# edp1096/toy-spice

Measured on NVIDIA B200. Metric: circuit-timesteps/sec (batched FP64 transient), higher is better.
Workload: dtype f64

## Files before the change

__graft_entry__.py:

```python
from __future__ import annotations

import importlib
import os
import re
import subprocess
import sys
from concurrent.futures import ThreadPoolExecutor

ROOT = os.path.dirname(os.path.abspath(__file__))
if ROOT not in sys.path:
    sys.path.insert(0, ROOT)

PKG = os.path.join(ROOT, "toy-spice_b200")
KCACHE = os.path.join(PKG, "_kcache")
NVCC = os.environ.get("NVCC", "/usr/local/cuda/bin/nvcc")
ARCH = ["-gencode", "arch=compute_100a,code=sm_100a"]


def _kernel_variants(T):
    W = importlib.import_module("toy-spice_b200.workloads")
    out = []

    def sweep_batch(ckt):
        b = ckt.batch(2)
        for (dev, par), vals in W.sweep_draws(ckt.devices(), 2, 1).items():
            b.set_param(dev, par, vals)
        return b

    for name, text in sorted(T.BUNDLED.items()):
        ckt = T.Circuit.from_netlist(text)
        out.append((name + ":nominal", ckt, ckt.batch(2)))
        out.append((name + ":sweep", ckt, sweep_batch(ckt)))
        card = ckt.analysis_card()
        if card["analysis"] == T.AN_DC:
            for label, b in ((":dc:nominal", ckt.batch(2)), (":dc:sweep", sweep_batch(ckt))):
                b.kernel_variant(card["dc_src_dev"])
                out.append((name + label, ckt, b))
    for k in (12, 24):
        ckt = T.Circuit.from_netlist(W.rc_ladder(k))
        out.append((f"ladder{k}:sweep", ckt, sweep_batch(ckt)))
    ckt = T.Circuit.from_netlist(W.diode_rc_ladder(24))
    out.append(("diodeladder24:sweep", ckt, sweep_batch(ckt)))
    try:
        sys.path.insert(0, os.path.join(ROOT, "tests"))
        extra = importlib.import_module("extra_decks").EXTRA
    except Exception:
        extra = {}
    for name, (text, an) in sorted(extra.items()):
        ckt = T.Circuit.from_netlist(text)
        out.append((name + ":sweep", ckt, sweep_batch(ckt)))
        if "dc" in an:
            cd = T.Circuit.from_netlist(an.get("dc_text", text))
            b = sweep_batch(cd)
            b.kernel_variant(an["dc"][0])
            out.append((name + ":dc:sweep", cd, b))
            if "dc_text" in an and an.get("op"):
                pass
        if "dc2" in an:
            b = sweep_batch(ckt)
            b.kernel_variant(an["dc2"][0][0], an["dc2"][1][0])
            out.append((name + ":dc2:sweep", ckt, b))
    try:
        acd = importlib.import_module("ac_decks")
        for name, text in sorted({**acd.AC_DECKS, **acd.AC_SINGULAR}.items()):
            ckt = T.Circuit.from_netlist(text)
            b = ckt.batch(2)
            for (dev, par), vals in acd.ac_draws(ckt.devices(), 2).items():
                b.set_param(dev, par, vals)
            out.append((name + ":ac", ckt, b))
    except Exception:
        pass
    return out

# ... 41 lines not shown
            break
    with open(os.path.join(KCACHE, autokey + ".auto"), "w") as f:
        f.write(f"{best}\n")
    return label, keys, status, best


def _coop_variants(T):
    out = []
    try:
        sys.path.insert(0, os.path.join(ROOT, "tests"))
        decks = dict(importlib.import_module("test_gpu_coop").DECKS)
        rd = importlib.import_module("random_decks")
        for k in (16,):
            decks[f"ladder{k}"] = (rd.rc_ladder(k), 0)
    except Exception as ex:
        print("[build] cooperative variants skipped:", ex)
        return out
    W = importlib.import_module("toy-spice_b200.workloads")
    for name, (text, _) in sorted(decks.items()):
        ckt = T.Circuit.from_netlist(text)
        b = ckt.batch(2)
        for (dev, par), vals in W.sweep_draws(ckt.devices(), 2, 1).items():
            b.set_param(dev, par, vals)
        out.append((f"{name}:thread:mb1", b, T.default_opts(strict_fp=0, min_blocks=1, coop_parts=0), ckt))
        for parts in (2, 4, 8):
            if ckt.coop_info(parts) is None:
                continue
            b = ckt.batch(2)
            for (dev, par), vals in W.sweep_draws(ckt.devices(), 2, 1).items():
                b.set_param(dev, par, vals)
            out.append((f"{name}:coop{parts}", b, T.default_opts(strict_fp=0, min_blocks=2, coop_parts=parts), ckt))
    ckt = T.Circuit.from_netlist(W.rc_ladder(32))
    b = ckt.batch(2)
    for (dev, par), vals in W.sweep_draws(ckt.devices(), 2, 1).items():
        b.set_param(dev, par, vals)
    out.append(("ladder32:thread:block96", b, T.default_opts(strict_fp=0, min_blocks=1, coop_parts=0, block_size=96), ckt))
    out.append(("ladder32:coop2", b, T.default_opts(strict_fp=0, min_blocks=2, coop_parts=2), ckt))
    return out


def _compile_coop(item):
    label, batch, opts, _ = item
    key = batch.kernel_key(opts)
    _, _, _, st = _nvcc_cubin(batch.kernel_source(opts), key, "true")
    return label, [key], st, 2


def build() -> None:
    subprocess.check_call(["make", "-C", os.path.join(PKG, "csrc"), "-s", "-j4"])
    T = importlib.import_module("toy-spice_b200")
    T.lib()
    os.makedirs(KCACHE, exist_ok=True)
    items = []
    seen = set()
    for label, ckt, batch in _kernel_variants(T):
        for strict in (0, 1):
            autokey = batch.kernel_key(T.default_opts(strict_fp=strict, min_blocks=0))
            if autokey in seen:
# ... 48 lines not shown
```

include/tspice_b200.h:

```cpp
#ifndef TSPICE_B200_H
#define TSPICE_B200_H

#include <stdint.h>

#ifdef __cplusplus
extern "C" {
#endif

typedef struct tsb_ctx tsb_ctx;
typedef struct tsb_plan tsb_plan;
typedef struct tsb_batch tsb_batch;
typedef struct tsb_job tsb_job;

enum {
    TSB_OK = 0,
    TSB_E_INVALID = -1,
    TSB_E_PARSE = -2,
    TSB_E_CUDA = -3,
    TSB_E_COMPILE = -4,
    TSB_E_UNSUPPORTED = -5,
    TSB_E_NOMEM = -6
};

enum {
// ... 129 lines not shown
int tsb_job_run_tran(tsb_job* job, double tstart, double tstop, double tstep, double tmax, int uic, int out_flags,
                     int64_t wave_cap_rows, const tsb_opts* opts);
int tsb_job_run_dc(tsb_job* job, int src_dev, double start, double stop, double inc, int out_flags, const tsb_opts* opts);
int tsb_job_sync(tsb_job* job);
int tsb_job_result_status(tsb_job* job, int32_t* status );
int tsb_job_result_rows(tsb_job* job, int64_t* rows );
int tsb_job_result_stats(tsb_job* job, double* stats );
int tsb_job_result_waveform(tsb_job* job, int64_t inst, double* out, int64_t cap_rows, int64_t* n_rows);
int tsb_job_result_summary(tsb_job* job, double* out, int64_t* rows_total, int64_t totals[5]);

int tsb_lu_order(int n, const double* A_nominal, int* pivot_row, int* pivot_col);
int tsb_batch_stamp_dev(tsb_batch* batch, int mode, double time, double dt, double gmin, uint64_t A_dev, uint64_t b_dev,
                        const tsb_opts* opts);
int tsb_lu_solve_batched(tsb_ctx* ctx, int n, const int* pivot_row, const int* pivot_col, const double* A, const double* b,
                         double* x, int32_t* status, int64_t n_inst, int strict_fp);
int tsb_lu_solve_batched_dev(tsb_ctx* ctx, int n, const int* pivot_row, const int* pivot_col, uint64_t A_dev, uint64_t b_dev,
                             uint64_t x_dev, uint64_t status_dev, int64_t n_inst, int strict_fp);
int tsb_lu_solve_batched_complex(tsb_ctx* ctx, int n, const int* pivot_row, const int* pivot_col, const double* A,
                                 const double* b, double* x, int32_t* status, int64_t n_inst, int strict_fp);
int tsb_lu_solve_batched_complex_dev(tsb_ctx* ctx, int n, const int* pivot_row, const int* pivot_col, uint64_t A_dev,
                                     uint64_t b_dev, uint64_t x_dev, uint64_t status_dev, int64_t n_inst, int strict_fp);

int tsb_batch_kernel_source(tsb_batch* batch, const tsb_opts* opts, char* buf, int64_t cap, int64_t* needed);
int tsb_batch_kernel_variant(tsb_batch* batch, int dc_src_dev, int dc_src2_dev, int grid);
int tsb_batch_kernel_key(tsb_batch* batch, const tsb_opts* opts, char* buf, int cap);
int64_t tsb_ctx_launch_count(const tsb_ctx* ctx);

#ifdef __cplusplus
}
#endif
#endif
```

toy-spice_b200/api.py:

```python
from __future__ import annotations

import ctypes as C
import os
import numpy as np

_HERE = os.path.dirname(os.path.abspath(__file__))
_LIB = None

AN_OP, AN_TRAN, AN_AC, AN_DC, AN_DC2 = 0, 1, 2, 3, 4
OUT_WAVE, OUT_STATS, OUT_GRID, OUT_AC_REFREAD = 1, 2, 4, 8
K_R, K_C, K_L, K_V, K_I, K_D, K_Q, K_M, K_K, K_LCORE = range(10)
ST_OK, ST_OP_FAILED, ST_TRAN_FAILED, ST_DC_FAILED, ST_OVERFLOW, ST_AC_FAILED = range(6)

ABI_SYMBOLS = [
    "tsb_default_opts", "tsb_version", "tsb_ctx_create", "tsb_ctx_destroy", "tsb_last_error", "tsb_ctx_set_stream",
    "tsb_ctx_set_cache_dir", "tsb_ctx_measure_fp64_peak", "tsb_ctx_sm_count", "tsb_plan_create",
    "tsb_plan_from_netlist", "tsb_plan_add_device", "tsb_plan_finalize", "tsb_plan_destroy", "tsb_plan_error",
    "tsb_plan_size", "tsb_plan_num_devices", "tsb_plan_device_info", "tsb_plan_device_params",
    "tsb_plan_find_device", "tsb_plan_node_name", "tsb_plan_analysis", "tsb_plan_structure", "tsb_plan_pattern",
    "tsb_plan_num_columns", "tsb_plan_column_name", "tsb_plan_coop_info", "tsb_batch_create", "tsb_batch_destroy", "tsb_batch_set_param",
    "tsb_batch_set_param_dev", "tsb_batch_set_param_uniform", "tsb_run_op", "tsb_run_tran", "tsb_run_dc",
    "tsb_batch_sync", "tsb_result_dims", "tsb_result_dev_ptrs", "tsb_result_rows", "tsb_result_status",
    "tsb_result_counters", "tsb_result_waveform", "tsb_result_wave_all", "tsb_result_stats_all",
    "tsb_result_totals", "tsb_batch_kernel_source", "tsb_batch_kernel_key", "tsb_ctx_launch_count",
# ... 402 lines not shown
        if np.isscalar(values):
            self._check(lib().tsb_batch_set_param_uniform(self.h, d, param, float(values)), "set_param_uniform")
            return
        if hasattr(values, "is_cuda") and values.is_cuda:
            import torch
            assert values.dtype == torch.float64 and values.is_contiguous() and values.numel() == self.n_inst
            self._keep[(d, param)] = values
            if self.ckt.ctx is not None:
                self.ckt.ctx.wait_torch_stream()
            self._check(lib().tsb_batch_set_param_dev(self.h, d, param, values.data_ptr()), "set_param_dev")
            return
        if hasattr(values, "numpy"):
            values = values.numpy()
        v = np.ascontiguousarray(values, dtype=np.float64)
        if v.shape != (self.n_inst,):
            raise ValueError("values must have shape [n_inst]")
        if zero_copy:
            self._keep[(d, param)] = v
            self._check(lib().tsb_batch_set_param_async(self.h, d, param, v.ctypes.data_as(C.POINTER(C.c_double))), "set_param_async")
        else:
            self._keep.pop((d, param), None)
            self._check(lib().tsb_batch_set_param(self.h, d, param, v.ctypes.data_as(C.POINTER(C.c_double))), "set_param")

    def kernel_variant(self, dc_src=-1, dc_src2=-1, grid=False):
        d1 = self._dev(dc_src) if dc_src != -1 else -1
        d2 = self._dev(dc_src2) if dc_src2 != -1 else -1
        self._check(lib().tsb_batch_kernel_variant(self.h, d1, d2, int(bool(grid))), "tsb_batch_kernel_variant")

    def kernel_source(self, opts: Opts | None = None) -> str:
        need = C.c_int64()
        o = C.byref(opts) if opts is not None else None
        lib().tsb_batch_kernel_source(self.h, o, None, 0, C.byref(need))
        buf = C.create_string_buffer(need.value)
        lib().tsb_batch_kernel_source(self.h, o, buf, need.value, C.byref(need))
        return buf.value.decode()

    def kernel_key(self, opts: Opts | None = None) -> str:
        buf = C.create_string_buffer(64)
        lib().tsb_batch_kernel_key(self.h, C.byref(opts) if opts is not None else None, buf, 64)
        return buf.value.decode()

    def run_op(self, opts: Opts | None = None):
        self._check(lib().tsb_run_op(self.h, C.byref(opts) if opts is not None else None), "tsb_run_op")

    def run_tran(self, tstart, tstop, tstep, tmax=0.0, uic=False, out=OUT_WAVE, cap_rows=0, opts: Opts | None = None):
        self._check(lib().tsb_run_tran(self.h, tstart, tstop, tstep, tmax, int(uic), out, cap_rows,
                                       C.byref(opts) if opts is not None else None), "tsb_run_tran")

    def run_dc(self, src, start, stop, inc, out=OUT_WAVE, opts: Opts | None = None):
        self._check(lib().tsb_run_dc(self.h, self._dev(src), start, stop, inc, out,
# ... 334 lines not shown
```

toy-spice_b200/csrc/codegen.cpp:

```cpp
#include <cstdio>
#include <algorithm>
#include <map>
#include <set>
#include <sstream>
#include <vector>
#include "tsb_internal.hpp"

namespace tsb {

static const char* k_models_src =
#include "models_src.inc"
    ;
static const char* k_skeleton_src =
#include "skeleton_src.inc"
    ;
static const char* k_coop_src =
#include "coop_src.inc"
    ;

namespace {

std::string dlit(double v) {
    char buf[64];
    if (v == (long long)v && v > -1e15 && v < 1e15) snprintf(buf, sizeof buf, "%lld.0", (long long)v);
// ... 833 lines not shown

void coop_dimensions(const Plan& pl, const CoopPlan& cp, int& nx, int& nown_max) {
    std::vector<CoopSym> sym;
    coop_analyse(pl, cp, sym, nx);
    nown_max = 0;
    for (const CoopSym& y : sym) nown_max = std::max(nown_max, (int)y.cols.size());
}

std::string generate_source(const Plan& pl, const CodegenConfig& cfg) {
    Emitter e;
    const int n = pl.n();
    const int ncol_tran = pl.num_columns(TSB_AN_TRAN);
    e.line("// Generated by tspice_b200 codegen: n=" + std::to_string(n) + ", " +
           std::to_string(pl.devs.size()) + " devices, " + std::to_string(pl.lu_main.pos.size()) + " matrix entries incl. fill" +
           (pl.lu_main.dense ? " (dense)" : "") + ".");
    e.line("#define TSB_BLOCK " + std::to_string(cfg.block_size));
    if (cfg.fast_div) e.line("#define TSB_FAST_DIV 1");
    e.line("#define TSB_MIN_BLOCKS " + std::to_string(cfg.min_blocks));
    e.line("#define TSB_SKIP_LINEAR_RESOLVE " + std::to_string(cfg.skip_linear ? 1 : 0));
    e.line("#define TSB_LANE_REFILL " + std::to_string(cfg.lane_refill && pl.has_nonlinear ? 1 : 0));
    e.line("#define TSB_GRID " + std::to_string(cfg.grid ? 1 : 0));
    e.line("#define TSB_ORDER " + std::to_string(cfg.order ? 1 : 0));
    e.line("#define TSB_TGRID " + std::to_string(cfg.tgrid && !pl.has_nonlinear && cfg.skip_linear ? 1 : 0));
    const CoopPlan* coop = nullptr;
    if (cfg.coop_parts > 0 && cfg.fast_div) { auto it = pl.coop.find(cfg.coop_parts); if (it != pl.coop.end()) coop = &it->second; }
    if (coop) e.line("#define TSB_COOP 1");
    if (!cfg.extra_defines.empty()) e.os << cfg.extra_defines << "\n";
    e.os << k_models_src << "\n" << k_skeleton_src << "\n";

    e.line("struct Ckt {");
    ++e.ind;
    e.line("static constexpr int N = " + std::to_string(n) + ";");
    e.line("static constexpr int NCOL_MAX = " + std::to_string(ncol_tran) + ";");
    e.line("static constexpr bool HAS_NL = " + std::string(pl.has_nonlinear ? "true" : "false") + ";");
    {
        bool uniform = true;
        for (const Dev& d : pl.devs)
            if (d.src_slot >= 0 && d.src_type() != TSB_SRC_PWL)
                for (size_t j = 0; j < d.p.size(); ++j) if (cfg.varying[d.p_off + (int)j]) uniform = false;
        e.line("static constexpr int NSRC = " + std::to_string(std::max(1, pl.n_src)) + ";");
        e.line("static constexpr bool SRC_UNIFORM = " + std::string(uniform ? "true" : "false") + ";");
    }
    e.line("static constexpr int DC_NESTED = " + std::string(cfg.dc_nested ? "1" : "0") + ";   // tsb_dc: rows carry SWEEP1 and SWEEP2 (dc.go:272-288)");
    e.line("double P[" + std::to_string(std::max(1, pl.n_params)) + "];      // parameters");
    e.line("double S[" + std::to_string(std::max(1, pl.n_state)) + "];      // device state carried between solves");
    e.line("double D[" + std::to_string(std::max(1, pl.n_derived)) + "];      // per-instance constants derived from P (1/R, L0, M)");
// ... 399 lines not shown
```

toy-spice_b200/csrc/device/skeleton.cuh:

```cuda
#ifndef TSB_SKELETON_CUH
#define TSB_SKELETON_CUH

#define TSB_MAX_VARYING 128
#define TSB_UC_MAX 32

struct TsbArgs {
    long long n_inst;
    const double* pv[TSB_MAX_VARYING];
    const double* U;
    int analysis;
    int uic;
    double tstart, tstop, tstep, maxstep, minstep;
    int max_iter;
    double abstol, reltol, trtol;
    int out_flags;
    long long cap_rows;
    double* wave;
    double* stats;
    long long* rows;
    int* status;
    long long* counters;
    double* scratch;
    const double* sweep;
    int n_sweep;
// ... 13 lines not shown
    double* coop_state;
};

__device__ __forceinline__ long long tsb_slot_instance(const TsbArgs& a, long long slot, bool valid) {
    return (TSB_ORDER && valid && a.order) ? a.order[slot] : slot;
}

#define TSB_ST_OK 0
#define TSB_ST_OP_FAILED 1
#define TSB_ST_TRAN_FAILED 2
#define TSB_ST_DC_FAILED 3
#define TSB_ST_OVERFLOW 4
#define TSB_AN_OP 0
#define TSB_AN_TRAN 1
#define TSB_AN_DC 3
#define TSB_OUT_WAVE 1
#define TSB_OUT_STATS 2
#define TSB_OUT_GRID 4
#define TSB_OUT_AC_REFREAD 8

#ifndef TSB_COOP
#define TSB_COOP 0
#endif
#ifndef TSB_X_STATS_PRED
#define TSB_X_STATS_PRED 1
#endif
#ifndef TSB_X_CONVSEL
#define TSB_X_CONVSEL 1
#endif
#ifndef TSB_X_LTE_OPAQUE
#define TSB_X_LTE_OPAQUE 1
#endif
#ifndef TSB_X_UNROLL2
#define TSB_X_UNROLL2 0
#endif
#ifndef TSB_X_TGLOOK
#define TSB_X_TGLOOK 1
#endif
#ifndef TSB_X_CONV2TOL
#define TSB_X_CONV2TOL 1
#endif
#ifndef TSB_X_NRSTATE
#define TSB_X_NRSTATE 1
#endif
#ifndef TSB_X_LTEFLAGS
#define TSB_X_LTEFLAGS 1
// ... 50 lines not shown
        }
    }
    __device__ __forceinline__ double grid_time(int k) const {
        const double t = __dadd_rn(a.tstart, __dmul_rn((double)(k + 1), a.grid_dt));
        return t < a.tstop ? t : a.tstop;
    }
    __device__ __forceinline__ void emit_grid(const double* row) {
        const double t1 = row[0];
        while (grid_k < a.n_grid) {
            const double tg = grid_time(grid_k);
            if (tg > t1) break;
            double w = 1.0;
            if (n_rows > 0) { const double t0 = sm[1 * TSB_BLOCK].y; w = (tg - t0) / (t1 - t0); }
            double* o = a.wave + ((long long)grid_k * NCOL) * a.n_inst + inst;
            __stcs(o, tg);
#pragma unroll
            for (int j = 1; j < NCOL; ++j) {
                const double v0 = n_rows > 0 ? sm[(2 * j + 1) * TSB_BLOCK].y : row[j];
                __stcs(o + j * a.n_inst, v0 + (row[j] - v0) * w);
            }
            ++grid_k;
        }
    }
    __device__ __forceinline__ void push(const double* row) {
        if (TSB_GRID && (a.out_flags & TSB_OUT_GRID)) emit_grid(row);
        if (a.out_flags & TSB_OUT_WAVE) {
            if (n_rows < a.cap_rows) {
                double* w = a.wave + (n_rows * NCOL) * a.n_inst + inst;
#pragma unroll
                for (int j = 0; j < NCOL; ++j) __stcs(w + j * a.n_inst, row[j]);
            } else overflow = true;
        }
        if (a.out_flags & TSB_OUT_STATS) {
            if (n_rows == 0) sm[0] = make_double2(row[0], row[0]);
            bool grow = !TSB_X_GROW;
#pragma unroll
            for (int j = 1; TSB_X_GROW && j < NCOL; ++j) {
                const double2 mm = sm[(2 * j) * TSB_BLOCK];
                grow |= (row[j] < mm.x) | (row[j] > mm.y);
            }
            if (grow) {
#pragma unroll
                for (int j = 1; j < NCOL; ++j) {
                    const double v = row[j];
                    double2 mm = sm[(2 * j) * TSB_BLOCK];
                    if (TSB_X_STATS_PRED) {
                        double* slot = reinterpret_cast<double*>(&sm[(2 * j) * TSB_BLOCK]);
                        if (v < mm.x) slot[0] = v;
                        if (v > mm.y) slot[1] = v;
                    } else {
                        mm.x = v < mm.x ? v : mm.x;
                        mm.y = v > mm.y ? v : mm.y;
                        sm[(2 * j) * TSB_BLOCK] = mm;
                    }
                }
            }
// ... 58 lines not shown
    asm volatile("ld.relaxed.gpu.global.u64 %0, [%1];" : "=l"(v) : "l"(p) : "memory");
    return v;
}
__device__ __forceinline__ void tsb_fence_acquire() { asm volatile("fence.acq_rel.gpu;" ::: "memory"); }
__device__ __forceinline__ void tsb_prefetch_l1(const void* p) { asm volatile("prefetch.global.L1 [%0];" ::"l"(p)); }
#ifndef TSB_TG_PUBLISH_EVERY
#define TSB_TG_PUBLISH_EVERY 8
#endif
#ifndef TSB_TG_LOOK_EVERY
#define TSB_TG_LOOK_EVERY 16
#endif
#ifndef TSB_TG_CACHED
#define TSB_TG_CACHED 0
#endif
#ifndef TSB_TG_PREFETCH
#define TSB_TG_PREFETCH 0
#endif
#if TSB_TG_CACHED
#define TSB_TG_LD(p) __ldca(p)
#else
#define TSB_TG_LD(p) __ldcg(p)
#endif

template <bool HAVE_KEY = false, bool HAVE_SMALL = false, class Ckt, class Sink>
__device__ __forceinline__ void tsb_accept_step(const TsbArgs& a, Ckt& c, Sink& sink, double& time, double& dt,
                                                double next_time, double lte, TsbTimeKeyer& keyer, double& last_key, double key_in = 0.0,
                                                bool lte_small = false) {
    c.load_state(dt);
    c.update_state();
    time = next_time;
    if (time >= a.tstart) {
        double key = HAVE_KEY ? key_in : keyer.key(time);
        if (key != last_key) {
            double row[Ckt::NCOL_MAX];
            row[0] = time;
            c.signals(row + 1);
            sink.push(row);
            last_key = key;
        }
    }
    if (time < a.tstop && dt < a.maxstep) {
        const double grown = (HAVE_SMALL ? lte_small : lte < a.trtol / 100) ? dt * 2 : dt * 1.1;
        dt = grown < a.maxstep ? grown : a.maxstep;
    }
}

template <class Ckt, class Sink>
__device__ __forceinline__ void tsb_tran_linear(const TsbArgs& a, Ckt& c, Sink& sink, long long& n_acc_out, long long& n_rej_out,
                                                long long& n_sol_tran_out, long long& n_exec_out, int& status, double& fail_at) {
    double time = 0.0, dt = a.minstep;
    double last_key = -1.0;
    TsbTimeKeyer keyer; keyer.reset();
    int n_acc = 0, n_rej = 0, n_bad = 0;
    constexpr int ND = TsbTgLayout<Ckt::NSRC>::ND;
    const bool tg_pub = TSB_TGRID && a.tgrid != nullptr && a.tgrid_role == 1;
    const bool tg_reader = TSB_TGRID && a.tgrid != nullptr && a.tgrid_role == 0;
    int tg_limit = TSB_X_TGLOOK ? 0 : (tg_reader ? 0 : -1);
    int tg_next = tg_reader ? 0 : 0x7fffffff;
#if TSB_X_UNROLL2
#pragma unroll 2
#endif
    while (time < a.tstop) {
        const int k = n_acc + n_rej;
        const double t_tag = time, dt_tag = dt;
        bool look = false;
        if (TSB_TGRID && TSB_X_TGLOOK) {
            if (k == tg_next) {
                const unsigned long long pub = tsb_ld_relaxed(a.tgrid_pub);
                const int lim = pub < (unsigned long long)a.tgrid_cap ? (int)pub : a.tgrid_cap;
                if (lim > k) { tsb_fence_acquire(); tg_limit = lim; tg_next = (lim + TSB_TG_LOOK_EVERY - 1) & ~(TSB_TG_LOOK_EVERY - 1); }
// ... 59 lines not shown
                    }
                }
            }
            if (!hit || !Ckt::SRC_UNIFORM) { if (!c.eval_sources_nb(time)) c.eval_sources(time, 1.0); }
            if (!hit) key = next_time >= a.tstart ? keyer.key_any(next_time) : -2.0;
            if (tg_pub && k < a.tgrid_cap) {
                double2* e = reinterpret_cast<double2*>(a.tgrid + (long long)k * ND);
                __stcg(e, make_double2(t_tag, dt_tag));
                __stcg(e + 1, make_double2(key, c.SV[0]));
#pragma unroll
                for (int j = 1; j < Ckt::NSRC; j += 2) __stcg(e + 2 + j / 2, make_double2(c.SV[j], j + 1 < Ckt::NSRC ? c.SV[j + 1] : 0.0));
                if ((k & (TSB_TG_PUBLISH_EVERY - 1)) == TSB_TG_PUBLISH_EVERY - 1) tsb_st_release(a.tgrid_pub, (unsigned long long)k + 1);
            }
        };
        bool solved;
        if constexpr (Ckt::HAS_TF) solved = c.template assemble_solve_tf<false>(time, dt, rdt, mid);
        else solved = c.template assemble_solve<TSB_MODE_TRAN, false>(TSB_MODE_TRAN, time, dt, rdt, 0.0, mid);
        if (!solved) {
            ++n_bad;
            if (dt > a.minstep) { dt /= 2; ++n_rej; continue; }
            status = TSB_ST_TRAN_FAILED; fail_at = time;
            break;
        }
        tsb_accept_step<true, true>(a, c, sink, time, dt, next_time, lte, keyer, last_key, key, lte_small);
        ++n_acc;
    }
    if (tg_pub) { const int k = n_acc + n_rej; tsb_st_release(a.tgrid_pub, (unsigned long long)(k < a.tgrid_cap ? k : a.tgrid_cap)); }
    n_acc_out += n_acc; n_rej_out += n_rej;
    const int failed = status == TSB_ST_TRAN_FAILED ? 1 : 0;
    n_exec_out += n_acc + (n_bad - failed) + failed;
    n_sol_tran_out += 2LL * (n_acc + n_rej) - n_bad + 2 * failed;
}

#ifndef TSB_X_NLLOOP
#define TSB_X_NLLOOP 1
#endif
template <class Ckt, class Sink>
__device__ __forceinline__ void tsb_tran_nonlinear(const TsbArgs& a, Ckt& c, Sink& sink, bool active, long long& n_acc_out,
                                                   long long& n_rej_out, long long& n_sol_tran_out, long long& n_exec_out,
                                                   int& status, double& fail_at) {
    constexpr int N = Ckt::N;
    double time = 0.0, dt = a.minstep;
    double last_key = -1.0;
    TsbTimeKeyer keyer; keyer.reset();
    int n_acc = 0, n_rej = 0, n_sol = 0;
    bool live = active && time < a.tstop;
    while (__any_sync(0xffffffffu, live)) {
// ... 262 lines not shown
                if (a.out_flags & TSB_OUT_WAVE) {
#pragma unroll
                    for (int i = 0; i < N; ++i) a.wave[(long long)i * a.n_inst + inst] = row[i];
                }
                sink.n_rows = 1;
                phase = PH_DONE;
            } else if (op_pass == 0) {
                op_pass = 1; status_dt = a.tstep; phase = PH_OP_START;
            } else {
                time = 0.0; dt = a.minstep;
                phase = time < a.tstop ? PH_TRAN_BEGIN : PH_DONE;
                if (LINEAR_LOOP || NL_LOOP) { linear_tran = true; phase = PH_DONE; }
            }
        }
    }
    if (LINEAR_LOOP) {
#if TSB_COOP
        if (a.coop_state) {
            if (linear_tran) c.dump_state(a.coop_state, a.n_inst, inst);
            finish_instance();
            return;
        }
#endif
        if (linear_tran) tsb_tran_linear(a, c, sink, n_acc, n_rej, n_sol_tran, n_exec, status, fail_at);
        finish_instance();
    }
    if (NL_LOOP) {
#if TSB_COOP
        if (a.coop_state) {
            if (valid) {
                if (linear_tran) c.dump_state(a.coop_state, a.n_inst, inst);
                finish_instance();
            }
            return;
        }
#endif
        tsb_tran_nonlinear(a, c, sink, valid && linear_tran, n_acc, n_rej, n_sol_tran, n_exec, status, fail_at);
        if (valid) finish_instance();
    }
}

template <class Ckt>
__device__ __forceinline__ void tsb_run_dc_instance(const TsbArgs& a, long long inst, bool valid) {
    constexpr int N = Ckt::N;
    constexpr int NC = Ckt::NCOL_MAX + Ckt::DC_NESTED;
    Ckt c;
    TsbSink<NC> sink(a, inst);
// ... 93 lines not shown
```

toy-spice_b200/csrc/runtime.cpp:

```cpp
#include <cuda_runtime.h>
#include <dlfcn.h>
#include <sys/stat.h>
#include <unistd.h>
#include <atomic>
#include <cmath>
#include <cstdio>
#include <cstdlib>
#include <cstring>
#include <fstream>
#include <memory>
#include <mutex>
#include <sstream>
#include "tsb_internal.hpp"
#include "hostlu.hpp"

namespace tsb {
cudaError_t launch_fp64_peak(double* scratch, int blocks, int iters, cudaStream_t s);
cudaError_t launch_totals(const long long* counters, long long n_inst, unsigned long long* totals, int sms, cudaStream_t s);
cudaError_t launch_fill_i64(long long* p, long long n, long long v, int sms, cudaStream_t s);
cudaError_t launch_summary(const double* stats, long long n_inst, int ncol, double* partial, int blocks_x, cudaStream_t s);
cudaError_t launch_lu_warp(const double* A, const double* b, double* x, int* status, long long n_inst, int n, const int* prow,
                           const int* pcol, int strict, int sms, cudaStream_t s);
cudaError_t launch_clu_warp(const double* A, const double* b, double* x, int* status, long long n_inst, int n, const int* prow,
                            const int* pcol, int strict, int sms, cudaStream_t s);
// ... 70 lines not shown
    std::atomic<int> refs{1};
};

struct tsb_batch {
    tsb_plan* plan = nullptr;
    tsb_ctx* ctx = nullptr;
    int64_t n_inst = 0;
    std::vector<double> uniform;
    std::vector<char> varying;
    std::vector<int> var_slot;
    std::vector<double*> slot_ptr;
    std::vector<char> slot_owned;
    std::vector<double*> slot_stage;
    std::vector<cudaEvent_t> slot_staged;
    double* d_uniform = nullptr;
    int analysis = -1, ncol = 0, out_flags = 0;
    int64_t cap_rows = 0;
    double *d_wave = nullptr, *d_stats = nullptr, *d_scratch = nullptr, *d_sweep = nullptr;
    long long *d_rows = nullptr, *d_counters = nullptr;
    int* d_status = nullptr;
    unsigned long long* d_totals = nullptr;
    unsigned long long* d_work = nullptr;
    bool grid_kernel = false;
    bool dc_nested = false;
    int dc_param2 = -1;
    double* d_sweep2 = nullptr;
    int intro_dc_param = -1;
    double* d_tgrid = nullptr;
    unsigned long long* d_tgrid_pub = nullptr;
    int tgrid_cap = 0, tgrid_nd = 0;
    int tgrid_used = 0;
    std::string tgrid_sig;
    cudaEvent_t ev_run = nullptr, ev_fetch = nullptr;
    cudaEvent_t ev_launched = nullptr, ev_params = nullptr;
    bool params_pending = false;
    bool fetch_pending = false;
    double* d_partial = nullptr;
    std::map<void*, size_t> guarded;
    std::string memo_sig, memo_autokey;
    KernelModule* memo_module = nullptr;
    long long* d_order = nullptr;
    double* d_coop_state = nullptr;
    size_t wave_bytes = 0, stats_bytes = 0;
};

namespace {
// ... 97 lines not shown
    }
    parse_ptxas_log(log, info);
    n = 0; g_nvrtc.GetCUBINSize(prog, &n);
    cubin.resize(n);
    g_nvrtc.GetCUBIN(prog, cubin.data());
    g_nvrtc.DestroyProgram(&prog);
    return n > 0;
}

CodegenConfig make_config(const tsb_batch* b, const tsb_opts& o, int dc_param) {
    CodegenConfig cfg;
    cfg.varying = b->varying; cfg.var_slot = b->var_slot; cfg.n_var = (int)b->slot_ptr.size();
    cfg.block_size = o.block_size > 0 ? o.block_size : 128;
    cfg.dc_param = dc_param;
    cfg.fast_div = !o.strict_fp;
    cfg.min_blocks = o.min_blocks;
    cfg.skip_linear = o.skip_linear_resolve != 0;
    cfg.lane_refill = o.lane_refill != 0;
    cfg.tgrid = o.share_time_grid != 0;
    cfg.coop_parts = o.coop_parts > 0 ? o.coop_parts : 0;
    if (cfg.coop_parts) cfg.tgrid = false;
    if (const char* tf = getenv("TSB_TRANFAST")) cfg.tranfast = *tf != '0';
    cfg.grid = b->grid_kernel;
    cfg.dc_nested = b->dc_nested; cfg.dc_param2 = b->dc_param2;
    cfg.order = b->d_order != nullptr;
    if (const char* x = getenv("TSB_EXTRA_DEFINES")) {
        std::string item;
        for (const char* c = x;; ++c) {
            if (*c == ';' || *c == '\0') {
                size_t eq = item.find('=');
                if (!item.empty()) {
                    std::string name = eq == std::string::npos ? item : item.substr(0, eq);
                    cfg.extra_defines += "#undef " + name + "\n#define " + name + " " + (eq == std::string::npos ? "1" : item.substr(eq + 1)) + "\n";
                }
                item.clear();
                if (*c == '\0') break;
            } else item += *c;
        }
    }
    return cfg;
}

bool read_file(const std::string& path, std::vector<char>& out) {
    std::ifstream f(path, std::ios::binary);
    if (!f) return false;
    out.assign(std::istreambuf_iterator<char>(f), std::istreambuf_iterator<char>());
// ... 18 lines not shown
    const std::string tmp = base + ".tmp" + std::to_string((long long)getpid());
    { std::ofstream f(tmp + ".cu"); f << src; }
    rename((tmp + ".cu").c_str(), (base + ".cu").c_str());
    if (!nvrtc_compile(src, base + ".cu", o, cubin, info, err)) return fail(ctx, TSB_E_COMPILE, err);
    { std::ofstream f(tmp + ".info"); f << info.regs << " " << info.spill_st << " " << info.spill_ld << "\n"; }
    rename((tmp + ".info").c_str(), (base + ".info").c_str());
    { std::ofstream f(tmp + ".cubin", std::ios::binary); f.write(cubin.data(), (std::streamsize)cubin.size()); }
    rename((tmp + ".cubin").c_str(), (base + ".cubin").c_str());
    return TSB_OK;
}

const int TSB_SPILL_OK = 100;
const int TSB_MAX_MIN_BLOCKS = 6;

int get_module_uncached(tsb_batch* b, tsb_opts o, int dc_param, KernelModule** out, std::string* autokey_out);

int get_module(tsb_batch* b, tsb_opts o, int dc_param, KernelModule** out, std::string* autokey_out = nullptr) {
    tsb_ctx* ctx = b->ctx;
    std::string sig;
    sig.reserve(b->varying.size() + 96);
    sig.append(b->varying.begin(), b->varying.end());
    const char* xd = getenv("TSB_EXTRA_DEFINES");
    char tail[200];
    snprintf(tail, sizeof tail, "|%d|%d|%d|%d|%d|%d|%d|%d|%d|%d|%d|%d|%lld|%p|", o.coop_parts, o.share_time_grid != 0, o.strict_fp, o.block_size, o.skip_linear_resolve, o.min_blocks, o.lane_refill,
             (int)b->grid_kernel, (int)(b->d_order != nullptr), dc_param, (int)b->dc_nested, b->dc_param2, ctx->choice_epoch, (void*)ctx);
    sig += tail;
    if (xd) sig += xd;
    if (const char* tf = getenv("TSB_TRANFAST")) { sig += "|tf"; sig += tf; }
    if (b->memo_module && sig == b->memo_sig) {
        *out = b->memo_module;
        if (autokey_out) *autokey_out = b->memo_autokey;
        return TSB_OK;
    }
    std::string autokey;
    const long long epoch0 = ctx->choice_epoch;
    int rc = get_module_uncached(b, o, dc_param, out, &autokey);
    if (rc != TSB_OK) return rc;
    if (autokey_out) *autokey_out = autokey;
    if (ctx->choice_epoch == epoch0) { b->memo_sig = sig; b->memo_autokey = autokey; b->memo_module = *out; }
    else b->memo_module = nullptr;
    return TSB_OK;
}

int get_module_uncached(tsb_batch* b, tsb_opts o, int dc_param, KernelModule** out, std::string* autokey_out) {
    tsb_ctx* ctx = b->ctx;
    std::vector<char> cubin;
    KernelInfo info;
    std::string src, key;
// ... 209 lines not shown
        r.block_size = (r.block_size + 31) / 32 * 32;
        if (r.block_size > 1024) r.block_size = 1024;
    }
    const char* env = getenv("TSB_STRICT_FP");
    if (env && *env) r.strict_fp = *env != '0';
    if (r.strict_fp < 0) r.strict_fp = plan.has_mutual ? 1 : 0;
    return r;
}

void fit_block_to_shared_memory(tsb_opts& o, int ncol, int out_flags) {
    if (!(out_flags & (TSB_OUT_STATS | TSB_OUT_GRID))) return;
    while (o.block_size > 32 && (size_t)4 * ncol * o.block_size * sizeof(double) > (size_t)226 * 1024) o.block_size -= 32;
}

const int64_t TSB_TUNE_MIN_INSTANCES = 1 << 15;

int autotune_min_blocks(tsb_batch* b, const tsb_opts& o_auto, const std::string& autokey, int rule_choice,
                        const TsbArgsHost& a_full, bool persistent) {
    tsb_ctx* ctx = b->ctx;
    const int block = o_auto.block_size > 0 ? o_auto.block_size : 128;
    cudaEvent_t e0, e1;
    CU(ctx, cudaEventCreate(&e0)); CU(ctx, cudaEventCreate(&e1));
    int best = rule_choice; double best_per = 0.0;
    for (int mb = rule_choice; mb <= TSB_MAX_MIN_BLOCKS && mb <= rule_choice + 2; ++mb) {
        tsb_opts o = o_auto; o.min_blocks = mb;
        KernelModule* m = nullptr;
        int rc = get_module(b, o, -1, &m);
        if (rc != TSB_OK) { cudaEventDestroy(e0); cudaEventDestroy(e1); return rc; }
        long long n_sub = (long long)ctx->sms * mb * block * 3;
        if (n_sub > b->n_inst) n_sub = b->n_inst;
        float ms = 0.f;
        for (int rep = 0; rep < 2; ++rep) {
            TsbArgsHost a = a_full; a.n_run = n_sub;
            CU(ctx, cudaEventRecord(e0, ctx->stream));
            if ((rc = launch(b, o, m->optran, a, persistent, m->min_blocks)) != TSB_OK) { cudaEventDestroy(e0); cudaEventDestroy(e1); return rc; }
            CU(ctx, cudaEventRecord(e1, ctx->stream));
            CU(ctx, cudaEventSynchronize(e1));
            CU(ctx, cudaEventElapsedTime(&ms, e0, e1));
        }
        const double per = (double)ms / (double)n_sub;
        if (mb == rule_choice || per < best_per * 0.97) { best = mb; best_per = per; }
    }
    cudaEventDestroy(e0); cudaEventDestroy(e1);
    ctx->auto_choice[autokey] = best;
    ++ctx->choice_epoch;
    ctx->tuned[autokey] = best;
    write_small_file(ctx->cache_dir + "/" + autokey + ctx->tuned_suffix, std::to_string(best) + "\n");
// ... 455 lines not shown
        const Plan& cpl = b->plan->p;
        o.coop_parts = 0;
        if (!cpl.has_bjt && !cpl.has_mutual && !o.strict_fp && !(out_flags & TSB_OUT_GRID) && o.skip_linear_resolve && !o.lane_refill) {
            if (cpl.n() >= TSB_COOP_AUTO_MIN_N)
                for (int pick : {2, 4, 8}) {
                    if (!cpl.coop.count(pick)) continue;
                    const int nx = cpl.coop.at(pick).nx, nown = cpl.coop.at(pick).nown_max;
                    if (((size_t)4 * nown * 32 * pick + (size_t)2 * pick * nx * 32) * sizeof(double) <= 110 * 1024) { o.coop_parts = pick; break; }
                }
        }
    }
    if (o.coop_parts != 0) {
        const Plan& cpl = b->plan->p;
        if (o.coop_parts != 2 && o.coop_parts != 4 && o.coop_parts != 8) return fail(ctx, TSB_E_INVALID, "coop_parts must be -1, 0, 2, 4 or 8");
        if (cpl.has_bjt || cpl.has_mutual) return fail(ctx, TSB_E_UNSUPPORTED, "coop_parts: circuits with BJTs or mutual couplings run thread-per-circuit");
        if (!cpl.coop.count(o.coop_parts)) return fail(ctx, TSB_E_UNSUPPORTED, "coop_parts: the netlist has no partition into that many sub-circuits (tsb_plan_coop_info)");
        if (o.strict_fp) return fail(ctx, TSB_E_UNSUPPORTED, "coop_parts: the nested-dissection order is a re-association, not available in the strict build");
        if (out_flags & TSB_OUT_GRID) return fail(ctx, TSB_E_UNSUPPORTED, "coop_parts: TSB_OUT_GRID is not available on the cooperative mapping");
        if (!o.skip_linear_resolve || o.lane_refill) return fail(ctx, TSB_E_UNSUPPORTED, "coop_parts needs skip_linear_resolve = 1 and lane_refill = 0");
        if (o.min_blocks <= 0) o.min_blocks = 2;
    } else fit_block_to_shared_memory(o, b->plan->p.num_columns(TSB_AN_TRAN), out_flags);
    KernelModule* m = nullptr;
    b->grid_kernel = (out_flags & TSB_OUT_GRID) != 0;
    std::string autokey;
    rc = get_module(b, o, -1, &m, &autokey);
    if (rc != TSB_OK) { b->grid_kernel = false; return rc; }
    if ((rc = alloc_results(b, TSB_AN_TRAN, out_flags, (out_flags & (TSB_OUT_WAVE | TSB_OUT_GRID)) ? wave_cap_rows : 0, 0)) != TSB_OK) return rc;
    TsbArgsHost a;
    if ((rc = fill_common(b, o, a)) != TSB_OK) return rc;
    a.analysis = TSB_AN_TRAN; a.uic = uic;
    a.tstart = tstart; a.tstop = tstop; a.tstep = tstep; a.maxstep = tmax; a.minstep = minstep;
    a.grid_dt = grid_dt; a.n_grid = (int)n_grid;
    const bool persistent = b->plan->p.has_nonlinear && o.lane_refill != 0;
    const char* tune_env = getenv("TSB_AUTOTUNE");
    cudaStreamCaptureStatus cap = cudaStreamCaptureStatusNone;
    if (cudaStreamIsCapturing(ctx->stream, &cap) != cudaSuccess) { cudaGetLastError(); cap = cudaStreamCaptureStatusNone; }
    if (o.coop_parts == 0 && o.min_blocks <= 0 && !autokey.empty() && b->n_inst >= TSB_TUNE_MIN_INSTANCES && !ctx->tuned.count(autokey) &&
        !(tune_env && *tune_env == '0') && cap == cudaStreamCaptureStatusNone) {
        rc = autotune_min_blocks(b, o, autokey, m->min_blocks, a, persistent);
        if (rc == TSB_OK) rc = get_module(b, o, -1, &m);
        if (rc != TSB_OK) { b->grid_kernel = false; return rc; }
    }
    b->grid_kernel = false;
    b->tgrid_used = 0;
    const Plan& pl = b->plan->p;
    if (o.coop_parts > 0) {
        if (!m->coop) return fail(ctx, TSB_E_COMPILE, "cooperative kernel missing from the module");
        const CoopPlan& cp = pl.coop.at(o.coop_parts);
        if (!b->d_coop_state) CU(ctx, cudaMalloc(&b->d_coop_state, (size_t)(pl.n_state + pl.n() + 1) * b->n_inst * sizeof(double)));
        a.coop_state = b->d_coop_state;
        TsbArgsHost a1 = a;
        a1.out_flags = 0;
        if ((rc = launch(b, o, m->optran, a1, false, m->min_blocks)) != TSB_OK) return rc;
        const int nx = cp.nx, nown = cp.nown_max;
        const int groups = 1, block = 32 * cp.parts * groups;
        const size_t smem = ((size_t)4 * nown * block + (size_t)groups * 2 * cp.parts * nx * 32) * sizeof(double);
        if (smem > 227 * 1024) return fail(ctx, TSB_E_UNSUPPORTED, "coop_parts: the statistics of one block do not fit in shared memory");
        if (smem > 48 * 1024) CU(ctx, cudaFuncSetAttribute((const void*)m->coop, cudaFuncAttributeMaxDynamicSharedMemorySize, (int)smem));
        long long blocks = (a.n_run + 32 * groups - 1) / (32 * groups);
        if (blocks > 0x7fffffffLL) blocks = 0x7fffffffLL;
        if (blocks < 1) blocks = 1;
        void* kargs[] = {&a};
        CU(ctx, cudaLaunchKernel((const void*)m->coop, dim3((unsigned)blocks), dim3((unsigned)block), kargs, smem, ctx->stream));
        ++ctx->launches;
        return note_launched(b);
    }
// ... 355 lines not shown
}

int tsb_lu_solve_batched_dev(tsb_ctx* ctx, int n, const int* pivot_row, const int* pivot_col, uint64_t A_dev, uint64_t b_dev,
                             uint64_t x_dev, uint64_t status_dev, int64_t n_inst, int strict_fp) {
    return lu_solve_dev(ctx, launch_lu_warp, n, pivot_row, pivot_col, A_dev, b_dev, x_dev, status_dev, n_inst, strict_fp);
}

int tsb_lu_solve_batched(tsb_ctx* ctx, int n, const int* pivot_row, const int* pivot_col, const double* A, const double* b,
                         double* x, int32_t* status, int64_t n_inst, int strict_fp) {
    return lu_solve_host(ctx, launch_lu_warp, 1, "tsb_lu_solve_batched", n, pivot_row, pivot_col, A, b, x, status, n_inst, strict_fp);
}

int tsb_lu_solve_batched_complex_dev(tsb_ctx* ctx, int n, const int* pivot_row, const int* pivot_col, uint64_t A_dev,
                                     uint64_t b_dev, uint64_t x_dev, uint64_t status_dev, int64_t n_inst, int strict_fp) {
    return lu_solve_dev(ctx, launch_clu_warp, n, pivot_row, pivot_col, A_dev, b_dev, x_dev, status_dev, n_inst, strict_fp);
}

int tsb_lu_solve_batched_complex(tsb_ctx* ctx, int n, const int* pivot_row, const int* pivot_col, const double* A,
                                 const double* b, double* x, int32_t* status, int64_t n_inst, int strict_fp) {
    return lu_solve_host(ctx, launch_clu_warp, 2, "tsb_lu_solve_batched_complex", n, pivot_row, pivot_col, A, b, x, status,
                         n_inst, strict_fp);
}

int tsb_batch_kernel_variant(tsb_batch* b, int dc_src_dev, int dc_src2_dev, int grid) {
    if (!b) return TSB_E_INVALID;
    const Plan& p = b->plan->p;
    auto param_of = [&](int d, int* out) {
        if (d < 0) { *out = -1; return true; }
        if (d >= (int)p.devs.size() || p.devs[d].kind != TSB_V) return false;
        const int st = p.devs[d].src_type();
        *out = (st == TSB_SRC_DC || st == TSB_SRC_SIN) ? p.devs[d].p_off : -1;
        return true;
    };
    int p1 = -1, p2 = -1;
    if (!param_of(dc_src_dev, &p1) || !param_of(dc_src2_dev, &p2)) return fail(b->ctx, TSB_E_INVALID, "source not found");
    b->intro_dc_param = p1; b->dc_param2 = p2; b->dc_nested = dc_src2_dev >= 0; b->grid_kernel = grid != 0;
    b->memo_module = nullptr;
    return TSB_OK;
}
int tsb_batch_kernel_source(tsb_batch* b, const tsb_opts* opts, char* buf, int64_t cap, int64_t* needed) {
    if (!b) return TSB_E_INVALID;
    tsb_opts o = resolve(opts, b->plan->p);
    std::string src = generate_source(b->plan->p, make_config(b, o, b->intro_dc_param));
    if (needed) *needed = (int64_t)src.size() + 1;
    if (buf && cap > 0) { snprintf(buf, (size_t)cap, "%s", src.c_str()); }
    return TSB_OK;
}
int tsb_batch_kernel_key(tsb_batch* b, const tsb_opts* opts, char* buf, int cap) {
    if (!b || !buf || cap < 33) return TSB_E_INVALID;
    tsb_opts o = resolve(opts, b->plan->p);
    std::string src = generate_source(b->plan->p, make_config(b, o, b->intro_dc_param));
    snprintf(buf, cap, "%s", source_key(src, compile_options_string(o)).c_str());
    return TSB_OK;
}

}
```

toy-spice_b200/csrc/tsb_internal.hpp:

```cpp
#pragma once
#include <cstdint>
#include <map>
#include <string>
#include <utility>
#include <vector>
#include "../../include/tspice_b200.h"

namespace tsb {

struct Dev {
    int kind = 0;
    std::string name;
    int nodes[4] = {0, 0, 0, 0};
    int n_nodes = 0;
    int branch = 0;
    std::vector<double> p;
    std::vector<int> ip;
    int p_off = 0;
    int s_off = 0, n_state = 0;
    int src_slot = -1;
    int d_off = -1;
    bool nonlinear() const { return kind == TSB_D || kind == TSB_Q || kind == TSB_M; }
    bool time_dependent() const { return kind == TSB_C || kind == TSB_L; }
    int src_type() const { return ip.empty() ? TSB_SRC_DC : ip[0]; }
// ... 81 lines not shown
    std::string column_name(int analysis_, int col) const;
};

int plan_from_netlist(const std::string& text, Plan& plan, std::string& err);
int plan_finalize(Plan& plan);
void device_stamp_entries(const Plan& plan, int dev_index, std::vector<StampEntry>& out);
struct AcEntry { int row, col, code; double sign; };
void device_ac_entries(const Plan& plan, int dev_index, std::vector<AcEntry>& out);
void ac_frequency_points(int sweep_type, int n_points, double fstart, double fstop, std::vector<double>& f);
int device_num_outputs(const Dev& d);
struct CodegenConfig {
    std::vector<char> varying;
    std::vector<int> var_slot;
    int n_var = 0;
    int block_size = 128;
    int dc_param = -1;
    int dc_param2 = -1;
    bool dc_nested = false;
    bool fast_div = false;
    int min_blocks = 1;
    bool skip_linear = true;
    std::string extra_defines;
    bool grid = false;
    bool order = false;
    bool lane_refill = false;
    bool tgrid = false;
    bool tranfast = true;
    int coop_groups = 1;
    int coop_parts = 0;
};
std::string generate_source(const Plan& plan, const CodegenConfig& cfg);
void coop_dimensions(const Plan& plan, const CoopPlan& cp, int& nx, int& nown_max);

}
```

Baseline: 122.3 billion.

## Specialize linear transient kernel for stats-only output and widen min-blocks autotune

Adds a stats-only kernel variant in which the output flags are fixed at compile time (TSB_OUT_FIXED). In the linear transient path this lets the compiler drop the wave and grid output branches and their register pressure. The runtime marks a batch as stats-only when the requested output is exactly stats, and includes that flag in the kernel cache key. The min_blocks autotuner now also tries rule_choice-1. The cost is an extra compiled variant per deck and a longer build.

```diff
diff --git a/__graft_entry__.py b/__graft_entry__.py
--- a/__graft_entry__.py
+++ b/__graft_entry__.py
@@ -27,18 +27,23 @@
             b.set_param(dev, par, vals)
         return b
 
+    def transient(label, ckt, make):
+        out.append((label, ckt, make(ckt)))
+        b = make(ckt)
+        b.kernel_variant(stats_only=True)
+        out.append((label + ":stats", ckt, b))
+
     for name, text in sorted(T.BUNDLED.items()):
         ckt = T.Circuit.from_netlist(text)
-        out.append((name + ":nominal", ckt, ckt.batch(2)))
-        out.append((name + ":sweep", ckt, sweep_batch(ckt)))
+        transient(name + ":nominal", ckt, lambda c: c.batch(2))
+        transient(name + ":sweep", ckt, sweep_batch)
         card = ckt.analysis_card()
         if card["analysis"] == T.AN_DC:
             for label, b in ((":dc:nominal", ckt.batch(2)), (":dc:sweep", sweep_batch(ckt))):
                 b.kernel_variant(card["dc_src_dev"])
                 out.append((name + label, ckt, b))
     for k in (12, 24):
-        ckt = T.Circuit.from_netlist(W.rc_ladder(k))
-        out.append((f"ladder{k}:sweep", ckt, sweep_batch(ckt)))
+        transient(f"ladder{k}:sweep", T.Circuit.from_netlist(W.rc_ladder(k)), sweep_batch)
     ckt = T.Circuit.from_netlist(W.diode_rc_ladder(24))
     out.append(("diodeladder24:sweep", ckt, sweep_batch(ckt)))
     try:
@@ -48,7 +53,7 @@
         extra = {}
     for name, (text, an) in sorted(extra.items()):
         ckt = T.Circuit.from_netlist(text)
-        out.append((name + ":sweep", ckt, sweep_batch(ckt)))
+        transient(name + ":sweep", ckt, sweep_batch)
         if "dc" in an:
             cd = T.Circuit.from_netlist(an.get("dc_text", text))
             b = sweep_batch(cd)
@@ -136,6 +141,7 @@
         b = ckt.batch(2)
         for (dev, par), vals in W.sweep_draws(ckt.devices(), 2, 1).items():
             b.set_param(dev, par, vals)
+        b.kernel_variant(stats_only=True)
         out.append((f"{name}:thread:mb1", b, T.default_opts(strict_fp=0, min_blocks=1, coop_parts=0), ckt))
         for parts in (2, 4, 8):
             if ckt.coop_info(parts) is None:
@@ -148,6 +154,7 @@
     b = ckt.batch(2)
     for (dev, par), vals in W.sweep_draws(ckt.devices(), 2, 1).items():
         b.set_param(dev, par, vals)
+    b.kernel_variant(stats_only=True)
     out.append(("ladder32:thread:block96", b, T.default_opts(strict_fp=0, min_blocks=1, coop_parts=0, block_size=96), ckt))
     out.append(("ladder32:coop2", b, T.default_opts(strict_fp=0, min_blocks=2, coop_parts=2), ckt))
     return out
diff --git a/include/tspice_b200.h b/include/tspice_b200.h
--- a/include/tspice_b200.h
+++ b/include/tspice_b200.h
@@ -175,7 +175,7 @@
                                      uint64_t b_dev, uint64_t x_dev, uint64_t status_dev, int64_t n_inst, int strict_fp);
 
 int tsb_batch_kernel_source(tsb_batch* batch, const tsb_opts* opts, char* buf, int64_t cap, int64_t* needed);
-int tsb_batch_kernel_variant(tsb_batch* batch, int dc_src_dev, int dc_src2_dev, int grid);
+int tsb_batch_kernel_variant(tsb_batch* batch, int dc_src_dev, int dc_src2_dev, int out);
 int tsb_batch_kernel_key(tsb_batch* batch, const tsb_opts* opts, char* buf, int cap);
 int64_t tsb_ctx_launch_count(const tsb_ctx* ctx);
 
diff --git a/toy-spice_b200/api.py b/toy-spice_b200/api.py
--- a/toy-spice_b200/api.py
+++ b/toy-spice_b200/api.py
@@ -448,10 +448,11 @@
             self._keep.pop((d, param), None)
             self._check(lib().tsb_batch_set_param(self.h, d, param, v.ctypes.data_as(C.POINTER(C.c_double))), "set_param")
 
-    def kernel_variant(self, dc_src=-1, dc_src2=-1, grid=False):
+    def kernel_variant(self, dc_src=-1, dc_src2=-1, grid=False, stats_only=False):
         d1 = self._dev(dc_src) if dc_src != -1 else -1
         d2 = self._dev(dc_src2) if dc_src2 != -1 else -1
-        self._check(lib().tsb_batch_kernel_variant(self.h, d1, d2, int(bool(grid))), "tsb_batch_kernel_variant")
+        out = 1 if grid else 2 if stats_only else 0
+        self._check(lib().tsb_batch_kernel_variant(self.h, d1, d2, out), "tsb_batch_kernel_variant")
 
     def kernel_source(self, opts: Opts | None = None) -> str:
         need = C.c_int64()
diff --git a/toy-spice_b200/csrc/codegen.cpp b/toy-spice_b200/csrc/codegen.cpp
--- a/toy-spice_b200/csrc/codegen.cpp
+++ b/toy-spice_b200/csrc/codegen.cpp
@@ -879,6 +879,7 @@
     e.line("#define TSB_GRID " + std::to_string(cfg.grid ? 1 : 0));
     e.line("#define TSB_ORDER " + std::to_string(cfg.order ? 1 : 0));
     e.line("#define TSB_TGRID " + std::to_string(cfg.tgrid && !pl.has_nonlinear && cfg.skip_linear ? 1 : 0));
+    if (cfg.stats_only && !pl.has_nonlinear && cfg.skip_linear && cfg.coop_parts == 0) e.line("#define TSB_OUT_FIXED TSB_OUT_STATS");
     const CoopPlan* coop = nullptr;
     if (cfg.coop_parts > 0 && cfg.fast_div) { auto it = pl.coop.find(cfg.coop_parts); if (it != pl.coop.end()) coop = &it->second; }
     if (coop) e.line("#define TSB_COOP 1");
diff --git a/toy-spice_b200/csrc/device/skeleton.cuh b/toy-spice_b200/csrc/device/skeleton.cuh
--- a/toy-spice_b200/csrc/device/skeleton.cuh
+++ b/toy-spice_b200/csrc/device/skeleton.cuh
@@ -59,6 +59,9 @@
 #ifndef TSB_COOP
 #define TSB_COOP 0
 #endif
+#ifndef TSB_OUT_FIXED
+#define TSB_OUT_FIXED -1
+#endif
 #ifndef TSB_X_STATS_PRED
 #define TSB_X_STATS_PRED 1
 #endif
@@ -155,16 +158,19 @@
             ++grid_k;
         }
     }
+    template <int OUT = -1>
+    __device__ __forceinline__ bool out(int f) const { return OUT >= 0 ? (OUT & f) != 0 && a.out_flags != 0 : (a.out_flags & f) != 0; }
+    template <int OUT = -1>
     __device__ __forceinline__ void push(const double* row) {
-        if (TSB_GRID && (a.out_flags & TSB_OUT_GRID)) emit_grid(row);
-        if (a.out_flags & TSB_OUT_WAVE) {
+        if (TSB_GRID && out<OUT>(TSB_OUT_GRID)) emit_grid(row);
+        if (out<OUT>(TSB_OUT_WAVE)) {
             if (n_rows < a.cap_rows) {
                 double* w = a.wave + (n_rows * NCOL) * a.n_inst + inst;
 #pragma unroll
                 for (int j = 0; j < NCOL; ++j) __stcs(w + j * a.n_inst, row[j]);
             } else overflow = true;
         }
-        if (a.out_flags & TSB_OUT_STATS) {
+        if (out<OUT>(TSB_OUT_STATS)) {
             if (n_rows == 0) sm[0] = make_double2(row[0], row[0]);
             bool grow = !TSB_X_GROW;
 #pragma unroll
@@ -269,7 +275,7 @@
 #define TSB_TG_LD(p) __ldcg(p)
 #endif
 
-template <bool HAVE_KEY = false, bool HAVE_SMALL = false, class Ckt, class Sink>
+template <bool HAVE_KEY = false, bool HAVE_SMALL = false, int OUT = -1, class Ckt, class Sink>
 __device__ __forceinline__ void tsb_accept_step(const TsbArgs& a, Ckt& c, Sink& sink, double& time, double& dt,
                                                 double next_time, double lte, TsbTimeKeyer& keyer, double& last_key, double key_in = 0.0,
                                                 bool lte_small = false) {
@@ -282,7 +288,7 @@
             double row[Ckt::NCOL_MAX];
             row[0] = time;
             c.signals(row + 1);
-            sink.push(row);
+            sink.template push<OUT>(row);
             last_key = key;
         }
     }
@@ -292,7 +298,7 @@
     }
 }
 
-template <class Ckt, class Sink>
+template <int OUT, class Ckt, class Sink>
 __device__ __forceinline__ void tsb_tran_linear(const TsbArgs& a, Ckt& c, Sink& sink, long long& n_acc_out, long long& n_rej_out,
                                                 long long& n_sol_tran_out, long long& n_exec_out, int& status, double& fail_at) {
     double time = 0.0, dt = a.minstep;
@@ -398,7 +404,7 @@
             status = TSB_ST_TRAN_FAILED; fail_at = time;
             break;
         }
-        tsb_accept_step<true, true>(a, c, sink, time, dt, next_time, lte, keyer, last_key, key, lte_small);
+        tsb_accept_step<true, true, OUT>(a, c, sink, time, dt, next_time, lte, keyer, last_key, key, lte_small);
         ++n_acc;
     }
     if (tg_pub) { const int k = n_acc + n_rej; tsb_st_release(a.tgrid_pub, (unsigned long long)(k < a.tgrid_cap ? k : a.tgrid_cap)); }
@@ -707,7 +713,7 @@
             return;
         }
 #endif
-        if (linear_tran) tsb_tran_linear(a, c, sink, n_acc, n_rej, n_sol_tran, n_exec, status, fail_at);
+        if (linear_tran) tsb_tran_linear<TSB_OUT_FIXED>(a, c, sink, n_acc, n_rej, n_sol_tran, n_exec, status, fail_at);
         finish_instance();
     }
     if (NL_LOOP) {
diff --git a/toy-spice_b200/csrc/runtime.cpp b/toy-spice_b200/csrc/runtime.cpp
--- a/toy-spice_b200/csrc/runtime.cpp
+++ b/toy-spice_b200/csrc/runtime.cpp
@@ -116,6 +116,7 @@
     unsigned long long* d_totals = nullptr;
     unsigned long long* d_work = nullptr;
     bool grid_kernel = false;
+    bool stats_kernel = false;
     bool dc_nested = false;
     int dc_param2 = -1;
     double* d_sweep2 = nullptr;
@@ -259,6 +260,7 @@
     if (cfg.coop_parts) cfg.tgrid = false;
     if (const char* tf = getenv("TSB_TRANFAST")) cfg.tranfast = *tf != '0';
     cfg.grid = b->grid_kernel;
+    cfg.stats_only = b->stats_kernel;
     cfg.dc_nested = b->dc_nested; cfg.dc_param2 = b->dc_param2;
     cfg.order = b->d_order != nullptr;
     if (const char* x = getenv("TSB_EXTRA_DEFINES")) {
@@ -323,8 +325,8 @@
     sig.append(b->varying.begin(), b->varying.end());
     const char* xd = getenv("TSB_EXTRA_DEFINES");
     char tail[200];
-    snprintf(tail, sizeof tail, "|%d|%d|%d|%d|%d|%d|%d|%d|%d|%d|%d|%d|%lld|%p|", o.coop_parts, o.share_time_grid != 0, o.strict_fp, o.block_size, o.skip_linear_resolve, o.min_blocks, o.lane_refill,
-             (int)b->grid_kernel, (int)(b->d_order != nullptr), dc_param, (int)b->dc_nested, b->dc_param2, ctx->choice_epoch, (void*)ctx);
+    snprintf(tail, sizeof tail, "|%d|%d|%d|%d|%d|%d|%d|%d|%d|%d|%d|%d|%d|%lld|%p|", o.coop_parts, o.share_time_grid != 0, o.strict_fp, o.block_size, o.skip_linear_resolve, o.min_blocks, o.lane_refill,
+             (int)b->grid_kernel, (int)b->stats_kernel, (int)(b->d_order != nullptr), dc_param, (int)b->dc_nested, b->dc_param2, ctx->choice_epoch, (void*)ctx);
     sig += tail;
     if (xd) sig += xd;
     if (const char* tf = getenv("TSB_TRANFAST")) { sig += "|tf"; sig += tf; }
@@ -580,7 +582,9 @@
     cudaEvent_t e0, e1;
     CU(ctx, cudaEventCreate(&e0)); CU(ctx, cudaEventCreate(&e1));
     int best = rule_choice; double best_per = 0.0;
-    for (int mb = rule_choice; mb <= TSB_MAX_MIN_BLOCKS && mb <= rule_choice + 2; ++mb) {
+    const int cand[4] = {rule_choice, rule_choice - 1, rule_choice + 1, rule_choice + 2};
+    for (int mb : cand) {
+        if (mb < 1 || mb > TSB_MAX_MIN_BLOCKS) continue;
         tsb_opts o = o_auto; o.min_blocks = mb;
         KernelModule* m = nullptr;
         int rc = get_module(b, o, -1, &m);
@@ -1082,9 +1086,10 @@
     } else fit_block_to_shared_memory(o, b->plan->p.num_columns(TSB_AN_TRAN), out_flags);
     KernelModule* m = nullptr;
     b->grid_kernel = (out_flags & TSB_OUT_GRID) != 0;
+    b->stats_kernel = out_flags == TSB_OUT_STATS;
     std::string autokey;
     rc = get_module(b, o, -1, &m, &autokey);
-    if (rc != TSB_OK) { b->grid_kernel = false; return rc; }
+    if (rc != TSB_OK) { b->grid_kernel = b->stats_kernel = false; return rc; }
     if ((rc = alloc_results(b, TSB_AN_TRAN, out_flags, (out_flags & (TSB_OUT_WAVE | TSB_OUT_GRID)) ? wave_cap_rows : 0, 0)) != TSB_OK) return rc;
     TsbArgsHost a;
     if ((rc = fill_common(b, o, a)) != TSB_OK) return rc;
@@ -1099,9 +1104,9 @@
         !(tune_env && *tune_env == '0') && cap == cudaStreamCaptureStatusNone) {
         rc = autotune_min_blocks(b, o, autokey, m->min_blocks, a, persistent);
         if (rc == TSB_OK) rc = get_module(b, o, -1, &m);
-        if (rc != TSB_OK) { b->grid_kernel = false; return rc; }
-    }
-    b->grid_kernel = false;
+        if (rc != TSB_OK) { b->grid_kernel = b->stats_kernel = false; return rc; }
+    }
+    b->grid_kernel = b->stats_kernel = false;
     b->tgrid_used = 0;
     const Plan& pl = b->plan->p;
     if (o.coop_parts > 0) {
@@ -1503,7 +1508,7 @@
                          n_inst, strict_fp);
 }
 
-int tsb_batch_kernel_variant(tsb_batch* b, int dc_src_dev, int dc_src2_dev, int grid) {
+int tsb_batch_kernel_variant(tsb_batch* b, int dc_src_dev, int dc_src2_dev, int out) {
     if (!b) return TSB_E_INVALID;
     const Plan& p = b->plan->p;
     auto param_of = [&](int d, int* out) {
@@ -1515,7 +1520,7 @@
     };
     int p1 = -1, p2 = -1;
     if (!param_of(dc_src_dev, &p1) || !param_of(dc_src2_dev, &p2)) return fail(b->ctx, TSB_E_INVALID, "source not found");
-    b->intro_dc_param = p1; b->dc_param2 = p2; b->dc_nested = dc_src2_dev >= 0; b->grid_kernel = grid != 0;
+    b->intro_dc_param = p1; b->dc_param2 = p2; b->dc_nested = dc_src2_dev >= 0; b->grid_kernel = out == 1; b->stats_kernel = out == 2;
     b->memo_module = nullptr;
     return TSB_OK;
 }
diff --git a/toy-spice_b200/csrc/tsb_internal.hpp b/toy-spice_b200/csrc/tsb_internal.hpp
--- a/toy-spice_b200/csrc/tsb_internal.hpp
+++ b/toy-spice_b200/csrc/tsb_internal.hpp
@@ -127,6 +127,7 @@
     bool skip_linear = true;
     std::string extra_defines;
     bool grid = false;
+    bool stats_only = false;
     bool order = false;
     bool lane_refill = false;
     bool tgrid = false;
```

Result: no change. 123.2 billion, median of 6 (+0.8%).
